# raymondfdavey/Conditioned-Diffusion-Models-UAD

Hardware: AMD Instinct MI355X
Metric: reconstructed 128x128 slices/sec @ T=1000 (higher is better)
Workload: dtype f32_emulated_f16x3

## Files before the change

### conditioned-diffusion-models-uad_amd/csrc/conv_x6.hip

```cpp
#include "kernels.h"
#include "conv_split.h"
#include <algorithm>
#include <cstdlib>
#include <cstring>
#include <type_traits>
#include <vector>

namespace cddpm {

static constexpr int ROWS = 8;
template <int TAPS, int NS, bool HI1 = false, int NB = 1>
__global__ __launch_bounds__(64 * ROWS) void conv_split_kernel(const ConvArgs a) {
    static_assert(NB == 1 || (NB == 2 && NS == 2 && TAPS != 1), "two cout blocks per workgroup: 16 x 16 fp16 form, LDS-DMA loop (3x3 and folded 2x2) only");
    typedef typename SplitT<NS>::v8 frag;
    constexpr int SP = 4 * NS;
    constexpr int THREADS = 64 * ROWS;
    constexpr bool UP2 = (TAPS == 4);
    constexpr int PAD = (TAPS == 9) ? 1 : 0;
    constexpr int PW = UP2 ? 33 : 32 + 2 * PAD;
    constexpr int PH = UP2 ? ROWS + 1 : ROWS + 2 * PAD;
    constexpr int NPIX = PW * PH;
    constexpr int NK = (NPIX * 8 + THREADS - 1) / THREADS;
    constexpr int FOLD = (TAPS == 9) ? 3 : (TAPS == 4 ? 2 : 1);
    constexpr int WSLOTS = 128 * SP;
    constexpr int TPS = (NS == 2) ? FOLD : 1;
    constexpr int WSTAGE = TPS * WSLOTS;
    constexpr int WK = WSLOTS / THREADS;
    static_assert(WSLOTS % THREADS == 0, "weight slab must divide evenly");

    extern __shared__ v4f lds[];
    v4f* ldsA = lds;
    v4f* ldsW = lds + NPIX * SP;
    v4f* ldsC = ldsW + 2 * WSTAGE;

    const int tid = threadIdx.x;
    const int lane = tid & 63;
    const int wave = tid >> 6;
    const int li = lane & 31;
    const int lh = lane >> 5;
    const int wm = wave % (ROWS / 2);
    const int wn = wave / (ROWS / 2);

    const int ncb = a.Cout >> 7;
    const int ncbw = ncb / NB;
    const int gridH = UP2 ? (a.H >> 1) : a.H, gridW = UP2 ? (a.W >> 1) : a.W;
    const int tilesX = (gridW + 31) >> 5;
    const int tilesY = (gridH + ROWS - 1) / ROWS;
    int bid = blockIdx.x;
    if ((gridDim.x & 7) == 0) bid = (blockIdx.x & 7) * (gridDim.x >> 3) + (blockIdx.x >> 3);
    const int cb = bid % ncbw;
    bid /= ncbw;
    const int nks = a.ksplit > 1 ? a.ksplit : 1;
    const int ks = bid % nks;
    bid /= nks;
    const int tx = bid % tilesX;
    bid /= tilesX;
    const int ty = bid % tilesY;
    bid /= tilesY;
    const int cls = UP2 ? (bid & 3) : 0;
    const int b = UP2 ? (bid >> 2) : bid;
    const int pa = cls >> 1, pb = cls & 1;
    const int y0 = ty * ROWS, x0 = tx * 32;

    auto slot_of = [](int row, int sp, int u) -> int {
        return (NS == 3) ? (row * 12 + 4 * sp + (u ^ ((row >> 2) & 3))) : (row * 8 + ((4 * sp + u) ^ ((row >> 1) & 7)));
    };
    constexpr bool M16 = (NS == 2);
    auto swz16 = [](int pc) -> int { return (2 * ((pc >> 1) & 3)) ^ (4 * (pc & 1)); };
    auto slot_a = [](int row, int sp, int u) -> int {
        if (NS == 3) return row * 12 + 4 * sp + (u ^ ((row >> 2) & 3));
        return row * 8 + ((4 * sp + u) ^ ((row >> 1) & 7) ^ (4 * (row & 1)));
    };

    const int Cin = a.C0 + a.C1;
    const int nch_main = Cin >> 5;
    const int nch_skip = (a.S0 + a.S1) >> 5;
    const int nch = nch_main + nch_skip;
    const int kc0 = a.ksplit > 1 ? a.kbound[ks] : 0;
    const int kc1 = a.ksplit > 1 ? a.kbound[ks + 1] : nch;

    const int c4 = tid & 7;
    int psrc[NK];
    unsigned centre = 0;
    unsigned colswz = 0;
#pragma unroll
    for (int k = 0; k < NK; ++k) {
        const int q = (tid >> 3) + (THREADS / 8) * k;
        const int pr = q / PW, pc = q - pr * PW;
        if constexpr (M16) colswz |= (unsigned)swz16(pc) << (3 * k);
        const int y = UP2 ? (y0 + pr + pa - 1) : (y0 + pr - PAD), x = UP2 ? (x0 + pc + pb - 1) : (x0 + pc - PAD);
        const bool valid = (q < NPIX) && (y >= 0) && (y < gridH) && (x >= 0) && (x < gridW);
        const int sy = (!UP2 && a.upsample) ? (y >> 1) : y, sx = (!UP2 && a.upsample) ? (x >> 1) : x;
        psrc[k] = valid ? (sy * a.srcW + sx) : -1;
        if (valid && (pr >= PAD) && (pr < PH - PAD) && (pc >= PAD) && (pc < PW - PAD)) centre |= 1u << k;
    }

    const v4f* wmain = reinterpret_cast<const v4f*>(a.wpk) + (size_t)(cls * ncb + NB * cb) * nch_main * TAPS * WSLOTS;
    const v4f* wskip = reinterpret_cast<const v4f*>(a.skip_wpk) + (size_t)(NB * cb) * nch_skip * WSLOTS;
    const size_t wmain_blk = (size_t)nch_main * TAPS * WSLOTS, wskip_blk = (size_t)nch_skip * WSLOTS;

    v4f wreg[WK];
    v4f areg[NK];
    const bool have_coef = (a.coef != nullptr);

    auto wslab = [&](int chunk, int tap) -> const v4f* {
        if (chunk >= nch) { chunk = 0; tap = 0; }
        return (chunk < nch_main) ? (wmain + ((size_t)chunk * TAPS + tap) * WSLOTS)
                                  : (wskip + (size_t)(chunk - nch_main) * WSLOTS);
    };
    auto load_act = [&](int chunk) {
        const float* base;
        int Cs, c0;
        const bool main_seg = chunk < nch_main;
        if (main_seg) {
            const int ch = chunk << 5;
            if (ch < a.C0) { base = a.src0; Cs = a.C0; c0 = ch; }
            else           { base = a.src1; Cs = a.C1; c0 = ch - a.C0; }
        } else {
            const int ch = (chunk - nch_main) << 5;
            if (ch < a.S0) { base = a.skip0; Cs = a.S0; c0 = ch; }
            else           { base = a.skip1; Cs = a.S1; c0 = ch - a.S0; }
        }
        const float* ubase = base + ((size_t)b * a.srcH * a.srcW * Cs + c0);
#pragma unroll
        for (int k = 0; k < NK; ++k) {
            const int p = (main_seg || ((centre >> k) & 1u)) ? psrc[k] : -1;
            v4f v = v4f{0.f, 0.f, 0.f, 0.f};
            if (p >= 0) v = *reinterpret_cast<const v4f*>(ubase + (__umul24((unsigned)p, (unsigned)Cs) + 4u * (unsigned)c4));
            areg[k] = v;
        }
    };
    typename SplitT<NS>::v4 sreg[NK][NS];
    auto transform_act = [&](int chunk) {
        const bool main_seg = chunk < nch_main;
        const bool do_silu = main_seg && a.silu;
        v4f cm = v4f{0.f, 0.f, 0.f, 0.f}, ca = v4f{1.f, 1.f, 1.f, 1.f}, cd = cm;
        const bool aff = main_seg && have_coef;
        if (aff) {
            const int ci = (chunk << 3) + c4;
            cm = ldsC[ci];
            ca = ldsC[(Cin >> 2) + ci];
            cd = ldsC[2 * (Cin >> 2) + ci];
        }
#pragma unroll
        for (int k = 0; k < NK; ++k) {
            v4f v = areg[k];
            const int p = (main_seg || ((centre >> k) & 1u)) ? psrc[k] : -1;
            if (p >= 0) {
                v = (v - cm) * ca + cd;
                if (do_silu) {
                    if constexpr (NS == 2) v = silu_x6_v4(v);
                    else { v.x = silu_x6(v.x); v.y = silu_x6(v.y); v.z = silu_x6(v.z); v.w = silu_x6(v.w); }
                }
            }
            split_x4<NS>(v, sreg[k]);
        }
    };
    auto write_act = [&]() {
        v2f* dst = reinterpret_cast<v2f*>(ldsA);
#pragma unroll
        for (int k = 0; k < NK; ++k) {
            const int q = (tid >> 3) + (THREADS / 8) * k;
            if (q < NPIX) {
#pragma unroll
                for (int sp = 0; sp < (HI1 ? 1 : NS); ++sp) {
                    const int sl = M16 ? (q * 8 + ((4 * sp + (c4 >> 1)) ^ (int)((colswz >> (3 * k)) & 7u))) : slot_a(q, sp, c4 >> 1);
                    dst[sl * 2 + (c4 & 1)] = __builtin_bit_cast(v2f, sreg[k][sp]);
                }
            }
        }
    };
    auto store_act = [&](int chunk) { transform_act(chunk); write_act(); };

    typedef float f32x4 __attribute__((ext_vector_type(4)));
    f32x16 acc[2][2], tot[2][2];
    f32x4 acc16[NB][4][4], tot16[4][4];
    if constexpr (M16) {
#pragma unroll
        for (int i = 0; i < 4; ++i)
#pragma unroll
            for (int j = 0; j < 4; ++j) {
                tot16[i][j] = f32x4{0.f, 0.f, 0.f, 0.f};
#pragma unroll
                for (int h = 0; h < NB; ++h) acc16[h][i][j] = tot16[i][j];
            }
    } else {
#pragma unroll
        for (int i = 0; i < 2; ++i)
#pragma unroll
            for (int j = 0; j < 2; ++j)
#pragma unroll
                for (int r = 0; r < 16; ++r) { acc[i][j][r] = 0.f; tot[i][j][r] = 0.f; }
    }
    auto fold_acc = [&]() {
        if constexpr (NB == 2) {
        } else if constexpr (M16) {
#pragma unroll
            for (int i = 0; i < 4; ++i)
#pragma unroll
                for (int j = 0; j < 4; ++j) tot16[i][j] += acc16[0][i][j];
        } else {
#pragma unroll
            for (int i = 0; i < 2; ++i)
#pragma unroll
                for (int j = 0; j < 2; ++j) tot[i][j] += acc[i][j];
        }
    };

    int brow[2];
#pragma unroll
    for (int nt = 0; nt < 2; ++nt) brow[nt] = 64 * wn + 32 * nt + li;

    constexpr int NKX = (TAPS == 9) ? 3 : (UP2 ? 2 : 1);
    static_assert(!M16 || TPS == NKX, "16x16 form: a weight stage is one row of taps, so the column shift is the unrolled index");
    int a_hi[NKX], a_mid[NKX], b_hi = 0, b_mid = 0;
    if constexpr (M16) {
        const int r16 = lane & 15, g = lane >> 4;
#pragma unroll
        for (int kx = 0; kx < NKX; ++kx) {
            const int pc = r16 + kx;
            a_hi[kx] = ((2 * wm) * PW + pc) * 8 + (g ^ swz16(pc));
            a_mid[kx] = a_hi[kx] ^ 4;
        }
        b_hi = slot_of(64 * wn + r16, 0, g);
        b_mid = b_hi ^ 4;
    }

    auto compute = [&](auto hc, int tap, int kxc, bool skip, const v4f* wb, bool first) {
        constexpr int HB = decltype(hc)::value;
        const f32x16 zero16 = {0.f, 0.f, 0.f, 0.f, 0.f, 0.f, 0.f, 0.f, 0.f, 0.f, 0.f, 0.f, 0.f, 0.f, 0.f, 0.f};
        const int ky = (TAPS == 9) ? (tap / 3) : (UP2 ? (tap >> 1) : 0);
        const int kx = (TAPS == 9) ? (tap - 3 * ky) : (UP2 ? (tap & 1) : 0);
        if constexpr (M16) {
            const f32x4 zero4 = {0.f, 0.f, 0.f, 0.f};
            f16x8 fa[2][4];
            const v4f* ah = ldsA + (((TAPS == 9 && skip) ? a_hi[NKX / 2] : a_hi[kxc]) + ky * (PW * 8));
            const v4f* am = ldsA + (((TAPS == 9 && skip) ? a_mid[NKX / 2] : a_mid[kxc]) + ky * (PW * 8));
            const v4f* bh = wb + b_hi;
            const v4f* bm = wb + b_mid;
#pragma unroll
            for (int t16 = 0; t16 < 4; ++t16) {
                const int off = ((t16 >> 1) * PW + (t16 & 1) * 16) * 8;
                fa[0][t16] = __builtin_bit_cast(f16x8, ah[off]);
                fa[1][t16] = __builtin_bit_cast(f16x8, am[off]);
            }
#pragma unroll
            for (int nh = 0; nh < 2; ++nh) {
                f16x8 fb[2][2];
#pragma unroll
                for (int j = 0; j < 2; ++j) {
                    fb[0][j] = __builtin_bit_cast(f16x8, bh[128 * (2 * nh + j)]);
                    fb[1][j] = __builtin_bit_cast(f16x8, bm[128 * (2 * nh + j)]);
                }
#pragma unroll
                for (int p = 0; p < 3; ++p) {
                    const int sa = (p == 0) ? 1 : 0, sb = (p == 1) ? 1 : 0;
                    if constexpr (HI1) { if (p < 2) continue; }
                    if ((HI1 ? p == 2 : p == 0) && first) {
#pragma unroll
                        for (int i = 0; i < 4; ++i)
#pragma unroll
                            for (int j = 0; j < 2; ++j)
                                acc16[HB][i][2 * nh + j] = __builtin_amdgcn_mfma_f32_16x16x32_f16(fa[sa][i], fb[sb][j], zero4, 0, 0, 0);
                    } else {
#pragma unroll
                        for (int i = 0; i < 4; ++i)
#pragma unroll
                            for (int j = 0; j < 2; ++j)
                                acc16[HB][i][2 * nh + j] = __builtin_amdgcn_mfma_f32_16x16x32_f16(fa[sa][i], fb[sb][j], acc16[HB][i][2 * nh + j], 0, 0, 0);
                    }
                }
            }
            return;
        }
        int arow[2];
#pragma unroll
        for (int mt = 0; mt < 2; ++mt) arow[mt] = (2 * wm + mt + ky) * PW + li + kx;
        constexpr int NP = (NS == 3) ? 6 : 3;
        constexpr int PA[6] = {NS == 3 ? 2 : 1, 0, 1, 1, 0, 0};
        constexpr int PB[6] = {0, NS == 3 ? 2 : 1, NS == 3 ? 1 : 0, 0, 1, 0};
#pragma unroll
        for (int jk = 0; jk < 2; ++jk) {
            const int u = 2 * jk + lh;
            frag fa[NS][2], fb[NS][2];
#pragma unroll
            for (int sp = 0; sp < NS; ++sp)
#pragma unroll
                for (int i = 0; i < 2; ++i) {
                    fa[sp][i] = __builtin_bit_cast(frag, ldsA[slot_a(arow[i], sp, u)]);
                    fb[sp][i] = __builtin_bit_cast(frag, wb[slot_of(brow[i], sp, u)]);
                }
#pragma unroll
            for (int p = 0; p < NP; ++p) {
                const int sa = (NS == 3) ? PA[p] : (p == 0 ? 1 : 0);
                const int sb = (NS == 3) ? PB[p] : (p == 1 ? 1 : 0);
                if (jk == 0 && p == 0 && first) {
#pragma unroll
                    for (int i = 0; i < 2; ++i)
#pragma unroll
                        for (int j = 0; j < 2; ++j) acc[i][j] = SplitT<NS>::mfma(fa[sa][i], fb[sb][j], zero16);
                } else {
#pragma unroll
                    for (int i = 0; i < 2; ++i)
#pragma unroll
                        for (int j = 0; j < 2; ++j) acc[i][j] = SplitT<NS>::mfma(fa[sa][i], fb[sb][j], acc[i][j]);
                }
            }
        }
    };

    if constexpr (TPS == 1) {
    {
        const v4f* p0 = wslab(kc0, 0);
#pragma unroll
        for (int i = 0; i < WK; ++i) wreg[i] = p0[tid + THREADS * i];
    }
    load_act(kc0);
    if (have_coef) {
        const int nq = Cin >> 2;
        const size_t plane = (size_t)a.B * Cin;
        for (int i = tid; i < 3 * nq; i += THREADS) {
            const int pl = i / nq, cq = i - pl * nq;
            ldsC[i] = *reinterpret_cast<const v4f*>(a.coef + pl * plane + (size_t)b * Cin + 4 * cq);
        }
    }
    int buf = 0;
    for (int chunk = kc0; chunk < kc1; ++chunk) {
        const bool main_seg = chunk < nch_main;
        const int ntap = main_seg ? TAPS : 1;
        __syncthreads();
        store_act(chunk);
        for (int t = 0; t < ntap; ++t) {
#pragma unroll
            for (int i = 0; i < WK; ++i) ldsW[buf * WSLOTS + tid + THREADS * i] = wreg[i];
            const bool last_tap = (t == ntap - 1);
            const v4f* pn = last_tap ? wslab(chunk + 1, 0) : wslab(chunk, t + 1);
#pragma unroll
            for (int i = 0; i < WK; ++i) wreg[i] = pn[tid + THREADS * i];
            if (last_tap && chunk + 1 < kc1) load_act(chunk + 1);
            __syncthreads();
            compute(std::integral_constant<int, 0>{}, main_seg ? t : (TAPS / 2), 0, !main_seg, ldsW + buf * WSLOTS, (t % FOLD) == 0);
            buf ^= 1;
            if ((t % FOLD) == FOLD - 1 || last_tap) fold_acc();
        }
    }

    } else {
    typedef const __attribute__((address_space(1))) void* gptr_t;
    typedef __attribute__((address_space(3))) void* lptr_t;
    auto wstage = [&](int chunk, int hb, int st, int& nsl) -> const v4f* {
        if (chunk < nch_main) { nsl = TPS; return wmain + hb * wmain_blk + ((size_t)chunk * TAPS + st * TPS) * WSLOTS; }
        nsl = 1;
        return wskip + hb * wskip_blk + (size_t)(chunk - nch_main) * WSLOTS;
    };
    static_assert(THREADS == 512 && WSLOTS == 1024, "one slab = 8 waves x 2 KB");
    auto dma_stage = [&](const v4f* p, int nsl, int buf) {
        const v4f* g0 = p + wave * 128 + lane;
        v4f* d0 = ldsW + buf * WSTAGE + wave * 128;
#pragma unroll
        for (int sl = 0; sl < TPS; ++sl)
            if (sl < nsl) {
                __builtin_amdgcn_global_load_lds((gptr_t)(g0 + sl * WSLOTS), (lptr_t)(d0 + sl * WSLOTS), 16, 0, 0);
                __builtin_amdgcn_global_load_lds((gptr_t)(g0 + sl * WSLOTS), (lptr_t)(d0 + sl * WSLOTS), 16, 1024, 0);
            }
    };
    int nsl_cur = 0;
    {
        const v4f* p0 = wstage(kc0, 0, 0, nsl_cur);
        dma_stage(p0, nsl_cur, 0);
    }
    load_act(kc0);
    if (have_coef) {
        const int nq = Cin >> 2;
        const size_t plane = (size_t)a.B * Cin;
        for (int i = tid; i < 3 * nq; i += THREADS) {
            const int pl = i / nq, cq = i - pl * nq;
            ldsC[i] = *reinterpret_cast<const v4f*>(a.coef + pl * plane + (size_t)b * Cin + 4 * cq);
        }
    }
    if (have_coef) __syncthreads();
    int buf = 0;
    for (int chunk = kc0; chunk < kc1; ++chunk) {
        const bool main_seg = chunk < nch_main;
        const int nst = main_seg ? TAPS / TPS : 1;
        asm volatile("s_waitcnt vmcnt(0)" ::: "memory");
        transform_act(chunk);
        __syncthreads();
        write_act();
        __syncthreads();
        if constexpr (NB == 1) {
        for (int st = 0; st < nst; ++st) {
            const int ntaps = nsl_cur;
            const bool last_st = (st == nst - 1);
            int nsl_next = 0;
            if (last_st && chunk + 1 < kc1) load_act(chunk + 1);
            if (!(last_st && chunk + 1 >= kc1)) {
                const v4f* pn = last_st ? wstage(chunk + 1, 0, 0, nsl_next) : wstage(chunk, 0, st + 1, nsl_next);
                dma_stage(pn, nsl_next, buf ^ 1);
            }
#pragma unroll
            for (int tt = 0; tt < TPS; ++tt)
                if (tt < ntaps) {
                    const int t = st * TPS + tt;
                    compute(std::integral_constant<int, 0>{}, main_seg ? t : (TAPS / 2), tt, !main_seg, ldsW + buf * WSTAGE + tt * WSLOTS, (t % FOLD) == 0);
                }
            buf ^= 1;
            nsl_cur = nsl_next;
            if (((st + 1) * TPS) % FOLD == 0 || last_st) fold_acc();
            if (!last_st) {
                asm volatile("s_waitcnt vmcnt(0)" ::: "memory");
                __syncthreads();
            }
        }
        } else {
        auto run_block = [&](auto hc) {
            constexpr int HB = decltype(hc)::value;
            for (int st = 0; st < nst; ++st) {
                const int ntaps = nsl_cur;
                const bool last_st = (st == nst - 1) && (HB == NB - 1);
                int nsl_next = 0;
                if (last_st && chunk + 1 < kc1) load_act(chunk + 1);
                if (!(last_st && chunk + 1 >= kc1)) {
                    const v4f* pn = last_st ? wstage(chunk + 1, 0, 0, nsl_next)
                                            : (st == nst - 1 ? wstage(chunk, HB + 1, 0, nsl_next) : wstage(chunk, HB, st + 1, nsl_next));
                    dma_stage(pn, nsl_next, buf ^ 1);
                }
#pragma unroll
                for (int tt = 0; tt < TPS; ++tt)
                    if (tt < ntaps) {
                        const int t = st * TPS + tt;
                        compute(hc, main_seg ? t : (TAPS / 2), tt, !main_seg, ldsW + buf * WSTAGE + tt * WSLOTS,
                                (NB == 1) && (t % FOLD) == 0);
                    }
                buf ^= 1;
                nsl_cur = nsl_next;
                if (((st + 1) * TPS) % FOLD == 0 || st == nst - 1) fold_acc();
                if (!last_st) {
                    asm volatile("s_waitcnt vmcnt(0)" ::: "memory");
                    __syncthreads();
                }
            }
        };
        run_block(std::integral_constant<int, 0>{});
        if constexpr (NB == 2) run_block(std::integral_constant<int, 1>{});
        }
    }

    }

    v4f rsd_all[2][2][4];
    auto load_rsd = [&](int q) {
        const int cq = lane & 7, prow = lane >> 3;
        const int hb = q >> 1, nt = q & 1;
#pragma unroll
        for (int hf = 0; hf < 2; ++hf)
#pragma unroll
            for (int i = 0; i < 4; ++i) {
                const int co = (NB * cb + hb) * 128 + 64 * wn + 32 * nt + 4 * cq;
                const int p = 8 * (4 * hf + i) + prow;
                const int gy = y0 + 2 * wm + (p >> 5), gx = x0 + (p & 31);
                const int y = UP2 ? (2 * gy + pa) : gy, x = UP2 ? (2 * gx + pb) : gx;
                v4f r = v4f{0.f, 0.f, 0.f, 0.f};
                if (a.res && (gy < gridH) && (gx < gridW)) {
                    const size_t rp = a.res_up ? ((size_t)(b * (a.H >> 1) + (y >> 1)) * (a.W >> 1) + (x >> 1))
                                               : ((size_t)(b * a.H + y) * a.W + x);
                    r = *reinterpret_cast<const v4f*>(a.res + rp * a.Cout + co);
                }
                rsd_all[q & 1][hf][i] = r;
            }
    };
    load_rsd(0);
    load_rsd(1);
    __syncthreads();
    {
        constexpr int TRS = M16 ? 36 : 32;
        float* tr = reinterpret_cast<float*>(lds) + wave * (64 * TRS);
        const int cq = lane & 7;
        const int prow = lane >> 3;
        const int tilesY4 = (gridH + 3) >> 2;
        const int ty4 = (y0 >> 2) + (wm >> 1);
#pragma unroll
        for (int q = 0; q < 2 * NB; ++q) {
            const int hb = q >> 1, nt = q & 1;
            const int co = (NB * cb + hb) * 128 + 64 * wn + 32 * nt + 4 * cq;
            if constexpr (M16) {
#pragma unroll
                for (int t16 = 0; t16 < 4; ++t16)
#pragma unroll
                    for (int n2 = 0; n2 < 2; ++n2)
#pragma unroll
                        for (int r = 0; r < 4; ++r)
                            tr[(16 * t16 + 4 * (lane >> 4) + r) * TRS + 16 * n2 + (lane & 15)] =
                                (NB == 2) ? acc16[hb][t16][2 * nt + n2][r] : tot16[t16][2 * nt + n2][r];
            } else {
#pragma unroll
                for (int mt = 0; mt < 2; ++mt)
#pragma unroll
                    for (int r = 0; r < 16; ++r)
                        tr[(mt * 32 + (r & 3) + 8 * (r >> 2) + 4 * lh) * 32 + li] = tot[mt][nt][r];
            }
            __builtin_amdgcn_wave_barrier();
            const v4f bias = a.bias ? *reinterpret_cast<const v4f*>(a.bias + co) : v4f{0.f, 0.f, 0.f, 0.f};
            const float wsc = (NS == 2) ? a.wscale_inv : 1.0f;
            v4f ssum = v4f{0.f, 0.f, 0.f, 0.f}, ssq = ssum;
#pragma unroll
            for (int hf = 0; hf < 2; ++hf) {
                v4f val[4];
                size_t oidx[4];
                bool ok[4];
#pragma unroll
                for (int i = 0; i < 4; ++i) {
                    const int p = 8 * (4 * hf + i) + prow;
                    const int gy = y0 + 2 * wm + (p >> 5), gx = x0 + (p & 31);
                    ok[i] = (gy < gridH) && (gx < gridW);
                    const int y = UP2 ? (2 * gy + pa) : gy, x = UP2 ? (2 * gx + pb) : gx;
                    oidx[i] = ((size_t)((ks * a.B + b) * a.H + y) * a.W + x) * a.Cout + co;
                    val[i] = *reinterpret_cast<const v4f*>(tr + p * TRS + 4 * cq);
                }
#pragma unroll
                for (int i = 0; i < 4; ++i)
                    if (ok[i]) {
                        const v4f o = val[i] * wsc + bias + rsd_all[q & 1][hf][i];
                        *reinterpret_cast<v4f*>(a.out + oidx[i]) = o;
                        ssum += o;
                        ssq += o * o;
                    }
            }
            if (q + 2 < 2 * NB) load_rsd(q + 2);
            if (a.stats) {
#pragma unroll
                for (int m = 8; m < 64; m <<= 1) {
                    ssum.x += __shfl_xor(ssum.x, m, 64); ssum.y += __shfl_xor(ssum.y, m, 64);
                    ssum.z += __shfl_xor(ssum.z, m, 64); ssum.w += __shfl_xor(ssum.w, m, 64);
                    ssq.x += __shfl_xor(ssq.x, m, 64); ssq.y += __shfl_xor(ssq.y, m, 64);
                    ssq.z += __shfl_xor(ssq.z, m, 64); ssq.w += __shfl_xor(ssq.w, m, 64);
                }
                if (prow == 0 && ty4 < tilesY4) {
                    const int nrec = (UP2 ? 8 : 2) * tilesX * tilesY4;
                    const int rec = 2 * ((cls * tilesY4 + ty4) * tilesX + tx) + (wm & 1);
                    float* o = a.stats + (((size_t)b * nrec + rec) * a.Cout + co) * 2;
                    *reinterpret_cast<v4f*>(o) = v4f{ssum.x, ssq.x, ssum.y, ssq.y};
                    *reinterpret_cast<v4f*>(o + 4) = v4f{ssum.z, ssq.z, ssum.w, ssq.w};
                }
            }
            __builtin_amdgcn_wave_barrier();
        }
    }
}

int conv_mode() {
    static const int mode = [] {
        const char* e = getenv("CDDPM_CONV");
        if (e && strcmp(e, "f32") == 0) return 0;
        if (e && strcmp(e, "x6") == 0) return 1;
        return 2;
    }();
    return mode;
}

template <int NS>
static void launch_split(const ConvArgs& a, hipStream_t stream) {
    const bool up2 = (a.taps == 4);
    const int gh = up2 ? a.H / 2 : a.H, gw = up2 ? a.W / 2 : a.W;
    const int tilesX = (gw + 31) / 32, tilesY = (gh + ROWS - 1) / ROWS;
    const bool nb2 = (NS == 2) && a.nb2 && a.ksplit <= 1 && (a.Cout % 256) == 0 && a.taps != 1;
    const unsigned grid = (unsigned)(a.B * (up2 ? 4 : 1) * tilesX * tilesY * (a.Cout / (nb2 ? 256 : 128)) * (a.ksplit > 1 ? a.ksplit : 1));
    const size_t coef_lds = a.coef ? (size_t)3 * (a.C0 + a.C1) * sizeof(float) : 0;
    const int npix = (a.taps == 9) ? (ROWS + 2) * 34 : (up2 ? (ROWS + 1) * 33 : ROWS * 32);
    const int tps = (NS == 2) ? (a.taps == 9 ? 3 : (up2 ? 2 : 1)) : 1;
    const size_t main = (size_t)(npix + 2 * tps * 128) * (4 * NS) * 16 + coef_lds;
    const size_t tr = (size_t)ROWS * 64 * 36 * sizeof(float);
    const size_t lds = main > tr ? main : tr;
    static bool attr = false;
    if (!attr) {
        (void)hipFuncSetAttribute(reinterpret_cast<const void*>(conv_split_kernel<9, NS>), hipFuncAttributeMaxDynamicSharedMemorySize, 160 * 1024);
        (void)hipFuncSetAttribute(reinterpret_cast<const void*>(conv_split_kernel<1, NS>), hipFuncAttributeMaxDynamicSharedMemorySize, 160 * 1024);
        (void)hipFuncSetAttribute(reinterpret_cast<const void*>(conv_split_kernel<4, NS>), hipFuncAttributeMaxDynamicSharedMemorySize, 160 * 1024);
        if constexpr (NS == 2) {
            (void)hipFuncSetAttribute(reinterpret_cast<const void*>(conv_split_kernel<9, NS, true>), hipFuncAttributeMaxDynamicSharedMemorySize, 160 * 1024);
            (void)hipFuncSetAttribute(reinterpret_cast<const void*>(conv_split_kernel<1, NS, true>), hipFuncAttributeMaxDynamicSharedMemorySize, 160 * 1024);
            (void)hipFuncSetAttribute(reinterpret_cast<const void*>(conv_split_kernel<4, NS, true>), hipFuncAttributeMaxDynamicSharedMemorySize, 160 * 1024);
            (void)hipFuncSetAttribute(reinterpret_cast<const void*>(conv_split_kernel<9, NS, false, 2>), hipFuncAttributeMaxDynamicSharedMemorySize, 160 * 1024);
            (void)hipFuncSetAttribute(reinterpret_cast<const void*>(conv_split_kernel<4, NS, false, 2>), hipFuncAttributeMaxDynamicSharedMemorySize, 160 * 1024);
            (void)hipFuncSetAttribute(reinterpret_cast<const void*>(conv_split_kernel<9, NS, true, 2>), hipFuncAttributeMaxDynamicSharedMemorySize, 160 * 1024);
            (void)hipFuncSetAttribute(reinterpret_cast<const void*>(conv_split_kernel<4, NS, true, 2>), hipFuncAttributeMaxDynamicSharedMemorySize, 160 * 1024);
        }
        attr = true;
    }
    const dim3 g(grid), blk(64 * ROWS);
    if constexpr (NS == 2) {
        if (nb2) {
            if (a.hi_only) {
                if (a.taps == 9) hipLaunchKernelGGL((conv_split_kernel<9, NS, true, 2>), g, blk, lds, stream, a);
                else hipLaunchKernelGGL((conv_split_kernel<4, NS, true, 2>), g, blk, lds, stream, a);
            } else if (a.taps == 9) hipLaunchKernelGGL((conv_split_kernel<9, NS, false, 2>), g, blk, lds, stream, a);
            else hipLaunchKernelGGL((conv_split_kernel<4, NS, false, 2>), g, blk, lds, stream, a);
            return;
        }
        if (a.hi_only) {
            if (a.taps == 9) hipLaunchKernelGGL((conv_split_kernel<9, NS, true>), g, blk, lds, stream, a);
            else if (a.taps == 1) hipLaunchKernelGGL((conv_split_kernel<1, NS, true>), g, blk, lds, stream, a);
            else hipLaunchKernelGGL((conv_split_kernel<4, NS, true>), g, blk, lds, stream, a);
            return;
        }
    }
    if (a.taps == 9) hipLaunchKernelGGL((conv_split_kernel<9, NS>), g, blk, lds, stream, a);
    else if (a.taps == 1) hipLaunchKernelGGL((conv_split_kernel<1, NS>), g, blk, lds, stream, a);
    else hipLaunchKernelGGL((conv_split_kernel<4, NS>), g, blk, lds, stream, a);
}

int conv_nb2_env() {
    static const int v = [] { const char* e = getenv("CDDPM_NB2"); return (e && e[0] == '0') ? 0 : (e && !strcmp(e, "force")) ? 2 : 1; }();
    return v;
}
bool conv_nb2_ok(int Cout, long long workgroups128, int ksplit, int family) {
    const int on = conv_nb2_env();
    return on && family == 2 && ksplit <= 1 && (Cout % 256) == 0 && (on == 2 || workgroups128 >= 512);
}

void launch_conv_split(const ConvArgs& a, hipStream_t stream) {
    if (a.family == 1) launch_split<3>(a, stream);
    else launch_split<2>(a, stream);
}

static inline uint16_t bf16_rne(float x) {
    uint32_t u;
    memcpy(&u, &x, 4);
    if ((u & 0x7f800000u) == 0x7f800000u) return (uint16_t)(u >> 16);
    u += 0x7fffu + ((u >> 16) & 1u);
    return (uint16_t)(u >> 16);
}
static inline float bf16_to_f(uint16_t h) {
    const uint32_t u = (uint32_t)h << 16;
    float f;
    memcpy(&f, &u, 4);
    return f;
}
static inline uint16_t f16_rne(float x) { const _Float16 h = (_Float16)x; uint16_t b; memcpy(&b, &h, 2); return b; }
static inline float f16_to_f(uint16_t b) { _Float16 h; memcpy(&h, &b, 2); return (float)h; }

int conv_weight_exp(const float* w, size_t n, int family) {
    if (family != 2) return 0;
    float mx = 0.f;
    for (size_t i = 0; i < n; ++i) { const float v = w[i] < 0 ? -w[i] : w[i]; if (v > mx) mx = v; }
    int e = 24;
    while (e > 0 && ldexpf(mx, e) >= 16384.0f) --e;
    return e;
}

void pack_conv_weights_split(const float* w, int Cout, int Cin, int taps, void* dst_, int wexp, int family) {
    uint16_t* dst = static_cast<uint16_t*>(dst_);
    const int ncb = Cout / 128, nch = Cin / 32;
    const int ns = (family == 1) ? 3 : 2, sp = 4 * ns;
    for (int cb = 0; cb < ncb; ++cb)
        for (int ch = 0; ch < nch; ++ch)
            for (int t = 0; t < taps; ++t) {
                uint16_t* img = dst + (((size_t)cb * nch + ch) * taps + t) * (128 * sp * 8);
                for (int j = 0; j < 128; ++j)
                    for (int u = 0; u < 4; ++u)
                        for (int e = 0; e < 8; ++e) {
                            const int co = cb * 128 + j, ci = ch * 32 + 8 * u + e;
                            float r = w[((size_t)co * Cin + ci) * taps + t];
                            if (ns == 3) {
                                for (int s3 = 0; s3 < 3; ++s3) {
                                    const uint16_t q = bf16_rne(r);
                                    r -= bf16_to_f(q);
                                    img[(size_t)(j * 12 + 4 * s3 + (u ^ ((j >> 2) & 3))) * 8 + e] = q;
                                }
                            } else {
                                r = ldexpf(r, wexp);
                                for (int s2 = 0; s2 < 2; ++s2) {
                                    const uint16_t q = f16_rne(r);
                                    r -= f16_to_f(q);
                                    img[(size_t)(j * 8 + ((4 * s2 + u) ^ ((j >> 1) & 7))) * 8 + e] = q;
                                }
                            }
                        }
            }
}

__device__ __forceinline__ void pack_split_unit(const float* __restrict__ w, int O, int I, int taps, int mode, int wexp,
                                                uint16_t* __restrict__ dst, long long id, int cls_in) {
    const int ncb = O / 128, nch = I / 32;
    if (id >= (long long)ncb * nch * taps * 512) return;
    const int u = (int)(id & 3), j = (int)((id >> 2) & 127);
    long long rest = id >> 9;
    const int t = (int)(rest % taps); rest /= taps;
    const int ch = (int)(rest % nch);
    const int cb = (int)(rest / nch);
    const int cls = cls_in;
    uint16_t* img = dst + ((((size_t)cls * ncb + cb) * nch + ch) * taps + t) * (size_t)(128 * 8 * 8);
    const int o = cb * 128 + j;
    union { uint16_t q[8]; uint4 v; } hi, mid;
    for (int e = 0; e < 8; ++e) {
        const int i = ch * 32 + 8 * u + e;
        float r;
        if (mode == 0) r = w[((size_t)o * I + i) * taps + t];
        else if (mode == 1) r = w[((size_t)i * O + o) * taps + (taps - 1 - t)];
        else {
            const int pa = cls >> 1, pb = cls & 1, ty = t >> 1, tx = t & 1;
            const int ky0 = pa == 0 ? (ty == 0 ? 0 : 1) : (ty == 0 ? 0 : 2), ky1 = pa == 0 ? (ty == 0 ? 0 : 2) : (ty == 0 ? 1 : 2);
            const int kx0 = pb == 0 ? (tx == 0 ? 0 : 1) : (tx == 0 ? 0 : 2), kx1 = pb == 0 ? (tx == 0 ? 0 : 2) : (tx == 0 ? 1 : 2);
            double acc = 0.0;
            for (int ky = ky0; ky <= ky1; ++ky)
                for (int kx = kx0; kx <= kx1; ++kx) acc += (double)w[((size_t)o * I + i) * 9 + ky * 3 + kx];
            r = (float)acc;
        }
        r = ldexpf(r, wexp);
        const _Float16 h = (_Float16)r;
        r -= (float)h;
        const _Float16 m = (_Float16)r;
        hi.q[e] = __builtin_bit_cast(uint16_t, h);
        mid.q[e] = __builtin_bit_cast(uint16_t, m);
    }
    const int sw = (j >> 1) & 7;
    *reinterpret_cast<uint4*>(img + (size_t)(j * 8 + ((0 + u) ^ sw)) * 8) = hi.v;
    *reinterpret_cast<uint4*>(img + (size_t)(j * 8 + ((4 + u) ^ sw)) * 8) = mid.v;
}
__global__ __launch_bounds__(256) void pack_split_kernel(const float* __restrict__ w, int O, int I, int taps, int mode, int wexp,
                                                         uint16_t* __restrict__ dst) {
    pack_split_unit(w, O, I, taps, mode, wexp, dst, (long long)blockIdx.x * 256 + threadIdx.x, (int)blockIdx.y);
}
__global__ __launch_bounds__(256) void pack_split_batch_kernel(const PackJob* __restrict__ jobs) {
    const PackJob j = jobs[blockIdx.y];
    pack_split_unit(j.w, j.O, j.I, j.taps, j.mode, j.wexp, static_cast<uint16_t*>(j.dst), (long long)blockIdx.x * 256 + threadIdx.x, j.cls);
}
void launch_pack_conv_split_batch(const PackJob* jobs_dev, int njobs, long long max_units, hipStream_t stream) {
    hipLaunchKernelGGL(pack_split_batch_kernel, dim3((unsigned)((max_units + 255) / 256), (unsigned)njobs), dim3(256), 0, stream, jobs_dev);
}
void launch_pack_conv_split(const float* w, int O, int I, int taps, int mode, int wexp, void* dst, hipStream_t stream) {
    const long long n = (long long)(O / 128) * (I / 32) * taps * 512;
    hipLaunchKernelGGL(pack_split_kernel, dim3((unsigned)((n + 255) / 256), mode == 2 ? 4 : 1), dim3(256), 0, stream, w, O, I, taps, mode, wexp,
                       static_cast<uint16_t*>(dst));
}

__global__ __launch_bounds__(256) void absmax_kernel(const float* __restrict__ x, long long n, unsigned* __restrict__ out) {
    unsigned m = 0;
    for (long long i = (long long)blockIdx.x * 256 + threadIdx.x; i < n; i += (long long)gridDim.x * 256)
        m = max(m, __float_as_uint(x[i]) & 0x7fffffffu);
    for (int o = 32; o > 0; o >>= 1) m = max(m, (unsigned)__shfl_xor((int)m, o));
    if ((threadIdx.x & 63) == 0 && m) atomicMax(out, m);
}
void launch_absmax(const float* x, long long n, float* out, hipStream_t stream) {
    (void)hipMemsetAsync(out, 0, sizeof(float), stream);
    const unsigned g = (unsigned)std::min<long long>((n + 255) / 256, 1024);
    hipLaunchKernelGGL(absmax_kernel, dim3(g), dim3(256), 0, stream, x, n, reinterpret_cast<unsigned*>(out));
}

}
```

Measured before the change: 1.454.

## Column-major activation fragments so MFMA tiles reuse A columns across taps

For the two-term fp16 split 3x3 and folded 2x2 convolutions with one cout block, activations are laid out in LDS by row with a padded pitch and column-parity swizzle. A new compute path walks consecutive pixel columns, so each horizontal tap reuses the previously loaded A fragments and loads only one new column per tap. The output transpose is remapped to match the new M ordering, which replaces per-wave barriers with workgroup barriers and adds a little LDS padding. The aim is fewer LDS reads per MFMA, at the cost of more complex indexing and extra synchronisation in the epilogue.

```diff
diff --git a/conditioned-diffusion-models-uad_amd/csrc/conv_x6.hip b/conditioned-diffusion-models-uad_amd/csrc/conv_x6.hip
--- a/conditioned-diffusion-models-uad_amd/csrc/conv_x6.hip
+++ b/conditioned-diffusion-models-uad_amd/csrc/conv_x6.hip
@@ -9,6 +9,9 @@
 namespace cddpm {
 
 static constexpr int ROWS = 8;
+static constexpr bool conv_colfrag(int ns, int taps, bool hi1, int nb) { return ns == 2 && taps != 1 && nb == 1; }
+static constexpr int conv_colfrag_pitch(int pw) { return pw * 8 + 2; }
+static constexpr int conv_colfrag_slots(int pw, int ph) { return (ph * conv_colfrag_pitch(pw) + 15) & ~15; }
 template <int TAPS, int NS, bool HI1 = false, int NB = 1>
 __global__ __launch_bounds__(64 * ROWS) void conv_split_kernel(const ConvArgs a) {
     static_assert(NB == 1 || (NB == 2 && NS == 2 && TAPS != 1), "two cout blocks per workgroup: 16 x 16 fp16 form, LDS-DMA loop (3x3 and folded 2x2) only");
@@ -28,9 +31,13 @@
     constexpr int WK = WSLOTS / THREADS;
     static_assert(WSLOTS % THREADS == 0, "weight slab must divide evenly");
 
+    constexpr bool COLF = conv_colfrag(NS, TAPS, HI1, NB);
+    constexpr int CPITCH = conv_colfrag_pitch(PW);
+    constexpr int ASLOTS = COLF ? conv_colfrag_slots(PW, PH) : NPIX * SP;
+
     extern __shared__ v4f lds[];
     v4f* ldsA = lds;
-    v4f* ldsW = lds + NPIX * SP;
+    v4f* ldsW = lds + ASLOTS;
     v4f* ldsC = ldsW + 2 * WSTAGE;
 
     const int tid = threadIdx.x;
@@ -87,7 +94,8 @@
     for (int k = 0; k < NK; ++k) {
         const int q = (tid >> 3) + (THREADS / 8) * k;
         const int pr = q / PW, pc = q - pr * PW;
-        if constexpr (M16) colswz |= (unsigned)swz16(pc) << (3 * k);
+        if constexpr (COLF) colswz |= (unsigned)(pr | ((pc & 1) << 4)) << (5 * k);
+        else if constexpr (M16) colswz |= (unsigned)swz16(pc) << (3 * k);
         const int y = UP2 ? (y0 + pr + pa - 1) : (y0 + pr - PAD), x = UP2 ? (x0 + pc + pb - 1) : (x0 + pc - PAD);
         const bool valid = (q < NPIX) && (y >= 0) && (y < gridH) && (x >= 0) && (x < gridW);
         const int sy = (!UP2 && a.upsample) ? (y >> 1) : y, sx = (!UP2 && a.upsample) ? (x >> 1) : x;
@@ -164,7 +172,8 @@
             if (q < NPIX) {
 #pragma unroll
                 for (int sp = 0; sp < (HI1 ? 1 : NS); ++sp) {
-                    const int sl = M16 ? (q * 8 + ((4 * sp + (c4 >> 1)) ^ (int)((colswz >> (3 * k)) & 7u))) : slot_a(q, sp, c4 >> 1);
+                    const int sl = COLF ? (q * 8 + 2 * (int)((colswz >> (5 * k)) & 15u) + ((4 * sp + (c4 >> 1)) ^ (4 * (int)((colswz >> (5 * k + 4)) & 1u))))
+                                 : M16 ? (q * 8 + ((4 * sp + (c4 >> 1)) ^ (int)((colswz >> (3 * k)) & 7u))) : slot_a(q, sp, c4 >> 1);
                     dst[sl * 2 + (c4 & 1)] = __builtin_bit_cast(v2f, sreg[k][sp]);
                 }
             }
@@ -213,9 +222,10 @@
 
     constexpr int NKX = (TAPS == 9) ? 3 : (UP2 ? 2 : 1);
     static_assert(!M16 || TPS == NKX, "16x16 form: a weight stage is one row of taps, so the column shift is the unrolled index");
-    int a_hi[NKX], a_mid[NKX], b_hi = 0, b_mid = 0;
+    int a_hi[NKX], a_mid[NKX], b_hi = 0, b_mid = 0, a_col = 0;
     if constexpr (M16) {
         const int r16 = lane & 15, g = lane >> 4;
+        a_col = (r16 & 7) * CPITCH + (4 * wm + 16 * (r16 >> 3)) * 8 + g;
 #pragma unroll
         for (int kx = 0; kx < NKX; ++kx) {
             const int pc = r16 + kx;
@@ -308,6 +318,50 @@
             }
         }
     };
+
+    auto compute_cols = [&](auto hc, auto kx0c, auto ntc, int ky, const v4f* wb) {
+        constexpr int HB = decltype(hc)::value, KX0 = decltype(kx0c)::value, NT = decltype(ntc)::value;
+        const f32x4 zero4 = {0.f, 0.f, 0.f, 0.f};
+        const v4f* ap = ldsA + (a_col + ky * CPITCH);
+        const v4f* bh = wb + b_hi;
+        const v4f* bm = wb + b_mid;
+        f16x8 fa[2][NT + 3];
+        auto read_col = [&](int c) {
+            const int pc = KX0 + c;
+            fa[0][c] = __builtin_bit_cast(f16x8, ap[pc * 8 + 4 * (pc & 1)]);
+            if constexpr (!HI1) fa[1][c] = __builtin_bit_cast(f16x8, ap[pc * 8 + 4 * ((pc & 1) ^ 1)]);
+        };
+#pragma unroll
+        for (int c = 0; c < 4; ++c) read_col(c);
+#pragma unroll
+        for (int tt = 0; tt < NT; ++tt) {
+            if (tt > 0) {
+                __builtin_amdgcn_sched_barrier(0);
+                read_col(tt + 3);
+            }
+#pragma unroll
+            for (int nh = 0; nh < 2; ++nh) {
+                f16x8 fb[2][2];
+#pragma unroll
+                for (int j = 0; j < 2; ++j) {
+                    fb[0][j] = __builtin_bit_cast(f16x8, bh[tt * WSLOTS + 128 * (2 * nh + j)]);
+                    if constexpr (!HI1) fb[1][j] = __builtin_bit_cast(f16x8, bm[tt * WSLOTS + 128 * (2 * nh + j)]);
+                }
+#pragma unroll
+                for (int p = 0; p < 3; ++p) {
+                    const int sa = (p == 0) ? 1 : 0, sb = (p == 1) ? 1 : 0;
+                    if constexpr (HI1) { if (p < 2) continue; }
+                    const bool first = (NB == 1) && (tt == 0) && (HI1 ? p == 2 : p == 0);
+#pragma unroll
+                    for (int i = 0; i < 4; ++i)
+#pragma unroll
+                        for (int j = 0; j < 2; ++j)
+                            acc16[HB][i][2 * nh + j] = __builtin_amdgcn_mfma_f32_16x16x32_f16(fa[sa][tt + i], fb[sb][j], first ? zero4 : acc16[HB][i][2 * nh + j], 0, 0, 0);
+                }
+            }
+        }
+    };
+    constexpr int SKY = (TAPS == 1) ? 0 : 1, SKX = (TAPS == 9) ? 1 : 0;
 
     if constexpr (TPS == 1) {
     {
@@ -398,6 +452,10 @@
                 const v4f* pn = last_st ? wstage(chunk + 1, 0, 0, nsl_next) : wstage(chunk, 0, st + 1, nsl_next);
                 dma_stage(pn, nsl_next, buf ^ 1);
             }
+            if constexpr (COLF) {
+                if (main_seg) compute_cols(std::integral_constant<int, 0>{}, std::integral_constant<int, 0>{}, std::integral_constant<int, TPS>{}, st, ldsW + buf * WSTAGE);
+                else compute_cols(std::integral_constant<int, 0>{}, std::integral_constant<int, SKX>{}, std::integral_constant<int, 1>{}, SKY, ldsW + buf * WSTAGE);
+            } else
 #pragma unroll
             for (int tt = 0; tt < TPS; ++tt)
                 if (tt < ntaps) {
@@ -425,6 +483,10 @@
                                             : (st == nst - 1 ? wstage(chunk, HB + 1, 0, nsl_next) : wstage(chunk, HB, st + 1, nsl_next));
                     dma_stage(pn, nsl_next, buf ^ 1);
                 }
+                if constexpr (COLF) {
+                    if (main_seg) compute_cols(hc, std::integral_constant<int, 0>{}, std::integral_constant<int, TPS>{}, st, ldsW + buf * WSTAGE);
+                    else compute_cols(hc, std::integral_constant<int, SKX>{}, std::integral_constant<int, 1>{}, SKY, ldsW + buf * WSTAGE);
+                } else
 #pragma unroll
                 for (int tt = 0; tt < TPS; ++tt)
                     if (tt < ntaps) {
@@ -474,7 +536,9 @@
     __syncthreads();
     {
         constexpr int TRS = M16 ? 36 : 32;
-        float* tr = reinterpret_cast<float*>(lds) + wave * (64 * TRS);
+        constexpr int TRW = 64 * TRS + (COLF ? 8 : 0);
+        float* tr = reinterpret_cast<float*>(lds) + wave * TRW;
+        float* trx = reinterpret_cast<float*>(lds) + (4 * wn + 2 * ((lane >> 4) & 1)) * TRW + (4 * wm + 16 * (lane >> 5)) * TRS + (lane & 15);
         const int cq = lane & 7;
         const int prow = lane >> 3;
         const int tilesY4 = (gridH + 3) >> 2;
@@ -483,7 +547,16 @@
         for (int q = 0; q < 2 * NB; ++q) {
             const int hb = q >> 1, nt = q & 1;
             const int co = (NB * cb + hb) * 128 + 64 * wn + 32 * nt + 4 * cq;
-            if constexpr (M16) {
+            if constexpr (COLF) {
+#pragma unroll
+                for (int t16 = 0; t16 < 4; ++t16)
+#pragma unroll
+                    for (int n2 = 0; n2 < 2; ++n2)
+#pragma unroll
+                        for (int r = 0; r < 4; ++r)
+                            trx[(r >> 1) * TRW + (32 * (r & 1) + t16) * TRS + 16 * n2] =
+                                (NB == 2) ? acc16[hb][t16][2 * nt + n2][r] : tot16[t16][2 * nt + n2][r];
+            } else if constexpr (M16) {
 #pragma unroll
                 for (int t16 = 0; t16 < 4; ++t16)
 #pragma unroll
@@ -499,7 +572,8 @@
                     for (int r = 0; r < 16; ++r)
                         tr[(mt * 32 + (r & 3) + 8 * (r >> 2) + 4 * lh) * 32 + li] = tot[mt][nt][r];
             }
-            __builtin_amdgcn_wave_barrier();
+            if constexpr (COLF) __syncthreads();
+            else __builtin_amdgcn_wave_barrier();
             const v4f bias = a.bias ? *reinterpret_cast<const v4f*>(a.bias + co) : v4f{0.f, 0.f, 0.f, 0.f};
             const float wsc = (NS == 2) ? a.wscale_inv : 1.0f;
             v4f ssum = v4f{0.f, 0.f, 0.f, 0.f}, ssq = ssum;
@@ -543,7 +617,8 @@
                     *reinterpret_cast<v4f*>(o + 4) = v4f{ssum.z, ssq.z, ssum.w, ssq.w};
                 }
             }
-            __builtin_amdgcn_wave_barrier();
+            if constexpr (COLF) { if (q + 1 < 2 * NB) __syncthreads(); }
+            else __builtin_amdgcn_wave_barrier();
         }
     }
 }
@@ -568,8 +643,9 @@
     const size_t coef_lds = a.coef ? (size_t)3 * (a.C0 + a.C1) * sizeof(float) : 0;
     const int npix = (a.taps == 9) ? (ROWS + 2) * 34 : (up2 ? (ROWS + 1) * 33 : ROWS * 32);
     const int tps = (NS == 2) ? (a.taps == 9 ? 3 : (up2 ? 2 : 1)) : 1;
-    const size_t main = (size_t)(npix + 2 * tps * 128) * (4 * NS) * 16 + coef_lds;
-    const size_t tr = (size_t)ROWS * 64 * 36 * sizeof(float);
+    const bool colf = conv_colfrag(NS, a.taps, a.hi_only, nb2 ? 2 : 1);    const int aslots = colf ? (a.taps == 9 ? conv_colfrag_slots(34, ROWS + 2) : conv_colfrag_slots(33, ROWS + 1)) : npix * 4 * NS;
+    const size_t main = (size_t)(aslots + 2 * tps * 128 * 4 * NS) * 16 + coef_lds;
+    const size_t tr = (size_t)ROWS * (64 * 36 + 8) * sizeof(float);
     const size_t lds = main > tr ? main : tr;
     static bool attr = false;
     if (!attr) {
```

After: 1.482, median of 6. 2.0% higher.
